# changhaonan/A3VLM

Hardware: AMD Instinct MI355X
Metric: image-text samples/sec (train) + articulation-decode tok/s (higher is better)
Workload: dtype bf16

## Files before the change

### a3vlm_amd/csrc/a3v_strip.hip

```cpp
#include "a3v_common.h"

namespace {
typedef __attribute__((ext_vector_type(4))) short s16x4;
constexpr int SBK = 64;
constexpr int SBN = 128;
constexpr int A_TILE = SBK * 128;
constexpr int W_TILE = SBK * 256;
constexpr int S_STAGE = A_TILE + W_TILE;

struct StripArgs {
  const bf16_t* T;
  const bf16_t* X;
  float* part;
  int64_t ldt, ldx;
  int R, N, Kt;
};

__device__ __forceinline__ int key_a(int k) { return (((k >> 3) & 1) << 1) | ((k >> 1) & 1); }
__device__ __forceinline__ int key_w(int k) { return (((k >> 3) & 1) << 2) | (k & 3); }

template <int NST>
__global__ __launch_bounds__(256) void gemm_tn_strip_kernel(StripArgs p) {
  __shared__ __attribute__((aligned(1024))) char lds[NST * S_STAGE];
  const int tid = threadIdx.x, lane = tid & 63;
  const int wave = __builtin_amdgcn_readfirstlane(tid >> 6);
  const int n0 = blockIdx.x * SBN;
  const int nk_all = (p.Kt + SBK - 1) / SBK;
  const int kt0 = (int)((int64_t)nk_all * blockIdx.y / gridDim.y), kt1 = (int)((int64_t)nk_all * (blockIdx.y + 1) / gridDim.y);
  const auto rsT = __builtin_amdgcn_make_buffer_rsrc((void*)p.T, 0, (int)(((int64_t)(p.Kt - 1) * p.ldt + 64) * 2), 0x00020000);
  const auto rsX = __builtin_amdgcn_make_buffer_rsrc((void*)p.X, 0, (int)(((int64_t)(p.Kt - 1) * p.ldx + p.N) * 2), 0x00020000);
  unsigned voT[2], voX[4];
#pragma unroll
  for (int c = 0; c < 2; ++c) {
    const int row = (wave * 2 + c) * 8 + (lane >> 3), pos = lane & 7;
    voT[c] = (unsigned)((row * p.ldt) * 2 + ((((pos >> 1) ^ key_a(row)) << 5) + (pos & 1) * 16));
  }
#pragma unroll
  for (int c = 0; c < 4; ++c) {
    const int row = (wave * 4 + c) * 4 + (lane >> 4), pos = lane & 15;
    voX[c] = (unsigned)((row * p.ldx) * 2 + ((((pos >> 1) ^ key_w(row)) << 5) + (pos & 1) * 16));
  }
  auto stage = [&](int t) {
    char* base = lds + ((t - kt0) % NST) * S_STAGE;
    const unsigned soT = (unsigned)(((int64_t)t * SBK * p.ldt) * 2);
    const unsigned soX = (unsigned)(((int64_t)t * SBK * p.ldx + n0) * 2);
#pragma unroll
    for (int c = 0; c < 2; ++c)
      __builtin_amdgcn_raw_ptr_buffer_load_lds(rsT, (__attribute__((address_space(3))) void*)(base + (wave * 2 + c) * 1024), 16, voT[c] + soT, 0, 0, 0);
#pragma unroll
    for (int c = 0; c < 4; ++c)
      __builtin_amdgcn_raw_ptr_buffer_load_lds(rsX, (__attribute__((address_space(3))) void*)(base + A_TILE + (wave * 4 + c) * 1024), 16, voX[c] + soX, 0, 0, 0);
  };
  const int fg = lane >> 4, il = lane & 15;
  int roA[2][2], kA[2][2], roW[2][2], kW[2][2];
#pragma unroll
  for (int ks = 0; ks < 2; ++ks)
#pragma unroll
    for (int jj = 0; jj < 2; ++jj) {
      const int k = ks * 32 + 8 * fg + 4 * jj + (il >> 2);
      roA[ks][jj] = k * 128 + (il & 3) * 8;
      kA[ks][jj] = key_a(k);
// ... 10 lines not shown
  };

  f32x4 acc[4][2];
#pragma unroll
  for (int i = 0; i < 4; ++i)
#pragma unroll
    for (int j = 0; j < 2; ++j) acc[i][j] = f32x4{0.f, 0.f, 0.f, 0.f};

  if (kt0 < kt1) stage(kt0);
  if (NST == 3 && kt0 + 1 < kt1) stage(kt0 + 1);
  for (int t = kt0; t < kt1; ++t) {
    if (NST == 3 && t + 1 < kt1) asm volatile("s_waitcnt vmcnt(6)" ::: "memory");
    else asm volatile("s_waitcnt vmcnt(0)" ::: "memory");
    __syncthreads();
    if (t + NST - 1 < kt1) stage(t + NST - 1);
    const char* At = lds + ((t - kt0) % NST) * S_STAGE;
    const char* Wt = At + A_TILE;
    bf16x8 af[2][4], wf[2][2];
#pragma unroll
    for (int ks = 0; ks < 2; ++ks) {
#pragma unroll
      for (int i = 0; i < 4; ++i) af[ks][i] = tr8(At, roA[ks][0], roA[ks][1], i ^ kA[ks][0], i ^ kA[ks][1]);
#pragma unroll
      for (int j = 0; j < 2; ++j) wf[ks][j] = tr8(Wt, roW[ks][0], roW[ks][1], (wave * 2 + j) ^ kW[ks][0], (wave * 2 + j) ^ kW[ks][1]);
    }
#pragma unroll
    for (int ks = 0; ks < 2; ++ks)
#pragma unroll
      for (int i = 0; i < 4; ++i)
#pragma unroll
        for (int j = 0; j < 2; ++j)
          acc[i][j] = __builtin_amdgcn_mfma_f32_16x16x32_bf16(wf[ks][j], af[ks][i], acc[i][j], 0, 0, 0);
  }
  float* plane = p.part + (int64_t)blockIdx.y * p.R * p.N;
#pragma unroll
  for (int i = 0; i < 4; ++i) {
    const int m = 16 * i + (lane & 15);
    if (m >= p.R) continue;
#pragma unroll
    for (int j = 0; j < 2; ++j) {
      const int n = n0 + 32 * wave + 16 * j + 4 * (lane >> 4);
      if (n + 4 <= p.N) *reinterpret_cast<f32x4*>(plane + (int64_t)m * p.N + n) = acc[i][j];
    }
  }
}
}

extern "C" int a3v_gemm_tn_strip(const void* T, int64_t ldt, const void* X, int64_t ldx, float* partial, int R, int N, int Kt, int S,
                                 void* stream) {
  if (!T || !X || !partial || R <= 0 || N <= 0 || Kt <= 0 || S < 1 || S > 64) return A3V_ERR_ARG;
  if (R > 64 || R % 4 || N % 4 || ldt % 8 || ldx % 8 || ldt < 64 || S > (Kt + SBK - 1) / SBK) return A3V_ERR_SHAPE;
  if (((int64_t)(Kt - 1) * ldt + 64) * 2 >= (1LL << 31) || ((int64_t)(Kt - 1) * ldx + N) * 2 >= (1LL << 31)) return A3V_ERR_SHAPE;
  if ((reinterpret_cast<uintptr_t>(T) | reinterpret_cast<uintptr_t>(X) | reinterpret_cast<uintptr_t>(partial)) & 15) return A3V_ERR_SHAPE;
  StripArgs p{(const bf16_t*)T, (const bf16_t*)X, partial, ldt, ldx, R, N, Kt};
  hipLaunchKernelGGL(gemm_tn_strip_kernel<2>, dim3((N + SBN - 1) / SBN, S), dim3(256), 0, (hipStream_t)stream, p);
  A3V_LAUNCH_CHECK();
  return A3V_OK;
}
```

### a3vlm_amd/lib.py

```python
from __future__ import annotations

import ctypes
import os
from ctypes import c_float, c_int, c_int64, c_void_p

_HERE = os.path.dirname(os.path.abspath(__file__))
LIB_PATH = os.environ.get("A3V_LIB_PATH") or os.path.join(_HERE, "liba3vlm_hip.so")

BF16, F32 = 0, 1
EPI_NONE, EPI_BIAS, EPI_GELU, EPI_QUICKGELU, EPI_RESIDUAL, EPI_SWIGLU, EPI_OUT_F32, EPI_RES_F32 = 0, 1, 2, 4, 8, 16, 32, 64
EPI_SWIGLU_BWD = 128

EPI_TILE_128, EPI_TILE_256, EPI_TILE_256PP = 1 << 16, 1 << 17, 1 << 18
EPI_TILE_192PP = 1 << 23

P, I, L, F = c_void_p, c_int, c_int64, c_float

SIGNATURES = {
    "a3v_version": (I, []),
    "a3v_reload_env": (I, []),
    "a3v_gemm_nt": (I, [P, L, P, L, P, L, I, I, I, P, P, L, I, I, P]),
    "a3v_gemm_qkv_rope": (I, [P, L, P, L, I, P, L, P, P, P, L, P, L, P, I, I, I, I, I, I, I, I, P]),
    "a3v_gemm_nt_fp8": (I, [P, L, P, P, L, P, P, L, I, I, I, P, P, L, I, P]),
    "a3v_gemm_qkv_rope_fp8": (I, [P, L, P, P, L, P, I, P, L, P, P, P, I, I, I, I, I, I, I, I, P]),
# ... 97 lines not shown
    "a3v_rope_kvcache_rows": (I, [P, L, P, L, P, P, P, P, I, I, I, I, I, I, P]),
    "a3v_attention_decode_rows": (I, [P, P, P, P, P, I, I, I, I, I, ctypes.POINTER(c_int64), P, P, I, P]),
    "a3v_attention_decode_rows_splits": (I, [I, I, I]),
    "a3v_attention_decode_rows_shared": (I, [P, P, P, P, P, P, P, I, I, I, I, I, ctypes.POINTER(c_int64), P, P, I, P]),
    "a3v_kv_copy_span": (I, [P, P, I, I, P, I, I, I, I, I, I, I, I, P]),
    "a3v_generate_step_rows": (I, [P, L, P, I, I, P, L, P, P, I, P, P, I, P, P, P, P, P, P]),
    "a3v_llama_decode_step_rows_form": (I, [I, I, I, I, I, I, I]),
    "a3v_rope_kvcache_spans": (I, [P, L, P, L, P, P, P, P, P, I, I, I, I, I, I, I, P]),
    "a3v_attention_verify_rows": (I, [P, P, P, P, P, P, I, I, I, I, I, I, ctypes.POINTER(c_int64), P, P, I, P]),
    "a3v_attention_verify_rows_splits": (I, [I, I, I]),
    "a3v_attention_verify_rows_scratch_floats": (L, [I, I, I, I, I]),
    "a3v_lookup_draft_rows": (I, [P, L, P, P, P, P, P, I, I, I, I, P, P, P]),
    "a3v_accept_rows": (I, [P, L, I, I, I, P, P, P, L, P, P, I, P, P, I, P, P, P, P, P, P]),
    "a3v_llama_decode_step_verify_form": (I, [I, I, I, I, I, I, I, I]),
    "a3v_seen_mark": (I, [P, L, P, P, L, I, I, P]),
    "a3v_seen_clear_rows": (I, [P, P, I, L, L, I, P]),
    "a3v_logits_prepare": (I, [P, L, P, L, F, P, L, P, I, I, P]),
    "a3v_generate_record": (I, [P, L, P, P, L, I, P, P, P, L, P, L, I, I, P, I, I, P]),
    "a3v_adam8_quantize": (I, [P, P, P, P, P, P, L, P]),
    "a3v_adam8_dequantize": (I, [P, P, P, P, P, P, L, P]),
    "a3v_adamw8_scaled": (I, [P, P, P, P, P, P, L, F, F, F, F, F, L, P, P, P]),
}

class LlamaLayer(ctypes.Structure):
    _fields_ = [(n, c_void_p) for n in ("attn_norm_w", "wqkv", "wo", "ffn_norm_w", "w13", "w2", "k_cache", "vt_cache",
                                        "wqkv_q", "wqkv_s", "wo_q", "wo_s", "w13_q", "w13_s", "w2_q", "w2_s",
                                        "wqkv_n4", "wqkv_n4s", "wo_n4", "wo_n4s", "w13_n4", "w13_n4s", "w2_n4", "w2_n4s")]


class Kv8Layer(ctypes.Structure):
    _fields_ = [(n, c_void_p) for n in ("k_q", "vt_q", "k_scale", "v_scale")]


class ImageDesc(ctypes.Structure):
    _fields_ = [("src", c_void_p), ("coeffs", c_void_p), ("bounds", c_void_p), ("H", c_int), ("W", c_int), ("side", c_int), ("pad_x", c_int),
                ("pad_y", c_int), ("ksize", c_int)]


SIGNATURES["a3v_llama_decode_step"] = (I, [ctypes.POINTER(LlamaLayer), I, P, P, P, P, P, P, P, P, I, I, I, I, I, I, I, I, F, P])
SIGNATURES["a3v_llama_decode_step_kv8"] = (I, [ctypes.POINTER(LlamaLayer), ctypes.POINTER(Kv8Layer), I, P, P, P, P, P, P, P, P, P, P,
                                               I, I, I, I, I, I, I, I, F, P])
SIGNATURES["a3v_llama_decode_step_form"] = (I, [I, I, I, I, I, I, I])
SIGNATURES["a3v_llama_decode_step_rows"] = (I, [ctypes.POINTER(LlamaLayer), I, P, P, P, P, P, P, P, P, P, I, I, I, I, I, I, I, I, F, P])
SIGNATURES["a3v_llama_decode_step_verify"] = (I, [ctypes.POINTER(LlamaLayer), I, P, P, P, P, P, P, P, P, P, P, I, I, I, I, I, I, I, I, I, F, P])
SIGNATURES["a3v_llama_decode_step_rows_shared"] = (I, [ctypes.POINTER(LlamaLayer), I, P, P, P, P, P, P, P, P, P, P, P, I, I, I, I, I, I, I, I,
                                                       F, P])

_lib = None


def load() -> ctypes.CDLL:
    global _lib
    if _lib is not None:
        return _lib
    if not os.path.isfile(LIB_PATH):
        raise RuntimeError(
            f"{LIB_PATH} not found: the HIP extension is not built. Run "
            "`python -c 'import __graft_entry__ as g; g.build()'` (or `make -C a3vlm_amd/csrc`). "
            "a3vlm_amd has no non-HIP fallback.")
    import torch
    lib = ctypes.CDLL(LIB_PATH)
    for name, (res, args) in SIGNATURES.items():
        fn = getattr(lib, name)
        fn.restype = res
        fn.argtypes = args
    _lib = lib
    return lib


class env:

    def __init__(self, **kw):
        self.kw = {k: str(v) for k, v in kw.items()}
        self.old = {}

    def __enter__(self):
        for k, v in self.kw.items():
            self.old[k] = os.environ.get(k)
            os.environ[k] = v
# ... 24 lines not shown
```

### a3vlm_amd/ops.py

```python
from __future__ import annotations

import ctypes
from typing import Optional

import torch

from . import lib as _l
from .lib import BF16, F32, EPI_BIAS, EPI_GELU, EPI_QUICKGELU, EPI_RESIDUAL, EPI_SWIGLU, EPI_OUT_F32, EPI_RES_F32, EPI_SWIGLU_BWD

_DT = {torch.bfloat16: BF16, torch.float32: F32}


def dt(t: torch.Tensor) -> int:
    try:
        return _DT[t.dtype]
    except KeyError:
        raise TypeError(f"a3vlm_amd supports bf16/fp32 tensors, got {t.dtype}")


def _p(t: Optional[torch.Tensor]):
    return None if t is None else t.data_ptr()


def _stream() -> int:
# ... 999 lines not shown


def grad_finish_multi(table, n_jobs: int, total_units: int, max_blocks: int = 0):
    _dev(table)
    assert table.dtype == torch.int64 and table.is_contiguous() and tuple(table.shape) == (n_jobs, 22)
    rc = _l.load().a3v_grad_finish_multi(_p(table), int(n_jobs), int(total_units), int(max_blocks), _stream())
    _l.check(rc, f"a3v_grad_finish_multi(jobs={n_jobs},units={total_units})")


def rmsnorm_bwd_parts(x, w, dy, dh, parts, eps, row_idx=None):
    _dev(x, w, dy, dh, parts, row_idx)
    assert w.dtype == torch.float32 and x.dtype == dh.dtype == dy.dtype == torch.bfloat16 and parts.dtype == torch.float32
    rows, dim = x.shape
    if row_idx is not None:
        assert row_idx.dtype == torch.int32 and row_idx.is_contiguous()
        rows = row_idx.numel()
        assert dy.shape[0] == rows
    assert parts.is_contiguous() and parts.numel() >= (rows + 7) // 8 * dim
    rc = _l.load().a3v_rmsnorm_bwd_parts_bf16(_p(x), x.stride(0), _p(row_idx), _p(w), _p(dy), dy.stride(0), _p(dh), dh.stride(0), _p(parts),
                                              rows, dim, eps, _stream())
    _l.check(rc, "a3v_rmsnorm_bwd_parts_bf16")


def gemm_tn_strip_planes(t, x, planes, S: int):
    _dev(t, x, planes)
    Kt, R = t.shape
    N = x.shape[1]
    assert x.shape[0] == Kt and t.stride(1) == 1 and x.stride(1) == 1 and t.stride(0) >= 64
    assert planes.dtype == torch.float32 and planes.is_contiguous() and planes.numel() >= S * R * N
    rc = _l.load().a3v_gemm_tn_strip(_p(t), t.stride(0), _p(x), x.stride(0), _p(planes), R, N, Kt, S, _stream())
    _l.check(rc, f"a3v_gemm_tn_strip(R={R},N={N},Kt={Kt},S={S})")


def lora_refresh(wa, wb, A, At, B, Bt, col0: int, row0: int):
    _dev(wa, wb, A, At, B, Bt)
    assert wa.dtype == torch.float32 and wb.dtype == torch.float32 and wa.is_contiguous() and wb.is_contiguous()
    assert all(t.dtype == torch.bfloat16 and t.stride(1) == 1 for t in (A, At, B, Bt))
    r, in_f = wa.shape
    nj = wb.shape[0]
    assert wb.shape[1] == r and col0 + r <= A.shape[0] and in_f <= A.shape[1] and row0 + nj <= B.shape[0]
    rc = _l.load().a3v_lora_refresh(_p(wa), _p(wb), r, in_f, nj, _p(A), A.stride(0), _p(At), At.stride(0), _p(B), B.stride(0), _p(Bt),
                                    Bt.stride(0), col0, row0, _stream())
    _l.check(rc, "a3v_lora_refresh")
```

### a3vlm_amd/train.py

```python
from __future__ import annotations

import os

from contextlib import contextmanager
from typing import Callable, Dict, List, Optional, Tuple

import torch

from . import grad_finish, ops
from .train_images import GROUPS, _AdapterImages, _Fp8Images, _Images, _Nf4Images, _pad64, group_modules
from .util import install_param_epoch_hook


def skinny_slices(M: int, N: int, K: int, cus: int) -> int:
    blocks = ((M + 127) // 128) * ((N + 127) // 128)
    nk = K // 64
    S = 1
    while blocks * S < 512 and S * 2 <= nk and S < 32:
        S *= 2
    if N <= 64 and M >= 2048 and cus > 0:
        S = max(1, min(cus // ((M + 255) // 256), nk // 2, 32))
    elif N <= 64 and M >= 512 and S > 4:
        S = 4
    return S


def label_rows_ref(labels: torch.Tensor, W: int, S: int):
    T = labels.shape[1]
    flat = labels.reshape(-1)
    pos = torch.nonzero(flat != 0).reshape(-1)
    b = torch.div(pos, T, rounding_mode="floor")
    return (b * S + W + (pos - b * T)).to(torch.int32), pos.to(torch.int32), flat[pos]


class TrainEngine:
    fuse_qkv_rope = os.environ.get("A3V_FUSE_QKV_ROPE", "1") != "0"
    tn_wgrad = os.environ.get("A3V_TN_WGRAD", "1") != "0"
    nn_dgrad = os.environ.get("A3V_NN_DGRAD", "1") != "0"
    packed_attn_bwd = os.environ.get("A3V_PACKED_ATTN_BWD", "1") != "0"
    lora_kext = os.environ.get("A3V_LORA_KEXT", "1") != "0"
    lora_nt_dgrad = os.environ.get("A3V_LORA_NT_DGRAD", "all")
    strip_wgrad = os.environ.get("A3V_STRIP_WGRAD", "1") != "0"
    fuse_swiglu_bwd = os.environ.get("A3V_FUSE_SWIGLU_BWD", "1") != "0"
    label_rows = os.environ.get("A3V_LABEL_ROWS", "1") != "0"
    finish_defer = os.environ.get("A3V_FINISH_DEFER", "1") != "0"
    finish_budget = int(float(os.environ.get("A3V_FINISH_BUDGET_MB", grad_finish.DEFAULT_BUDGET // 2 ** 20)) * 2 ** 20)

    def __init__(self, model, compute_dtype: torch.dtype = torch.bfloat16, recompute: Optional[bool] = None,
                 stream_dtype: Optional[torch.dtype] = None, zero1_world: int = 0):
        install_param_epoch_hook()
        self.m = model
        self.lora = int(getattr(model, "lora_rank", 0) or 0) > 0
        self.act = compute_dtype
        if stream_dtype is None:
            stream_dtype = torch.float32 if os.environ.get("A3V_STREAM_FP32", "0") == "1" else compute_dtype
        self.stream = stream_dtype
        self.recompute = recompute
        self._img = None
        self._ws: Dict[tuple, torch.Tensor] = {}
        self._flat: Optional[torch.Tensor] = None
        self._views: Dict[str, torch.Tensor] = {}
        self._ranges: List[Tuple[str, int, int]] = []
        self._fresh: set = set()
        self._gemm_written: set = set()
        self.on_layer_grads_ready: Optional[Callable[[str, int, int], None]] = None
        self.sumsq_sink = None
        self.static_grad_scale: Optional[float] = None
        self._saved = None
        self._weights_ready: Dict[str, torch.cuda.Event] = {}
        self.zero1_world = int(zero1_world or 0)
        if "A3V_NN_DGRAD" not in os.environ:
            self.nn_dgrad = bool(self.zero1_world)
        if self._q4base() and self.zero1_world:
            raise ValueError("ZeRO-1 shards compute-dtype base matrices; an NF4 base (quantize_base_weights) has none")
        if self._q8base():
            if self.zero1_world:
                raise ValueError("ZeRO-1 shards compute-dtype base matrices; an fp8 base (quantize_base_weights) has none")
            if compute_dtype != torch.bfloat16:
                raise ValueError(f"an fp8 base trains under the bf16 compute dtype (the products of its GEMMs are bf16); got {compute_dtype}")
        self._flat_params: Optional[torch.Tensor] = None
        self._z1: List[tuple] = []
        self._z1_fresh = True
        self._params: Dict[str, torch.nn.Parameter] = {}
        self._offs: Dict[str, Tuple[int, int]] = {}
        self._adapters = _AdapterImages(self)
        self._cu_count: Optional[int] = None
        self._nt_mem_checked = False
        self._opt_stepped = False
        self._dha_ready = False
        self._dh_full: Optional[torch.Tensor] = None
        self._sel_rows: Optional[Tuple[int, int]] = None
        self.bucket_overlap = False
        self._fin: Optional[grad_finish.GradFinisher] = None
        self._fin_mode: Optional[str] = None
        self._fin_hold: Optional[List[str]] = None

    def _buf(self, name, shape, dtype=None, zero=False):
        dtype = dtype or self.act
        if self._sel_rows is not None:
            return self._sel_buf(name, tuple(shape), dtype, zero)
        key = (name, tuple(shape), dtype)
        t = self._ws.get(key)
        if t is None:
            t = torch.empty(*shape, dtype=dtype, device=self.m._device)
            self._ws[key] = t
        if zero:
            t.zero_()
        return t

    def _sel_buf(self, name, shape, dtype, zero):
        n, cap = self._sel_rows
        name += ".sel"
        if shape[0] == n:
            key = (name, (cap,) + shape[1:], dtype)
            t = self._ws.get(key)
            if t is None:
                t = self._ws[key] = torch.empty(*key[1], dtype=dtype, device=self.m._device)
            t = t[:n]
        else:
            numel = 1
            for d in shape:
                numel *= d
            key = (name, "flat", dtype)
            t = self._ws.get(key)
            if t is None or t.numel() < numel:
                t = self._ws[key] = torch.empty(numel, dtype=dtype, device=self.m._device)
            t = t[:numel].view(shape)
        if zero:
# ... 260 lines not shown
        if tn_ok and self._strip_ok(dy, x):
            S = self._strip_slices(M, K)
            ops.gemm_tn_strip(dy, x, grad, self._buf("splitk", (S * N * K,), torch.float32), S, accumulate=not fresh)
            return
        if tn_ok and min(N, K) <= 64 and max(N, K) >= 256:
            blocks = ((N + 255) // 256) * ((K + 255) // 256)
            S = 1
            while blocks * S < 256 and S < 16 and 2 * S <= (M + 63) // 64:
                S *= 2
            ops.gemm_tn_splitk(dy, x, grad, self._buf("splitk", (S * N * K,), torch.float32), S, accumulate=not fresh)
            return
        Mp = _pad64(M)
        dyt = self._buf("wg_dyt" + tag, (N, Mp))
        xt = self._buf("wg_xt" + tag, (K, Mp))
        ops.transpose(dy, dyt, M, N, Mp)
        ops.transpose(x, xt, M, K, Mp)
        if min(N, K) <= 64:
            self._skinny(dyt, xt, grad, accumulate=not fresh)
        else:
            ops.gemm_nt(dyt, xt, grad, residual=None if fresh else grad,
                        epilogue=(ops.EPI_OUT_F32 if fresh else ops.EPI_RES_F32) if self.act == torch.bfloat16 else 0)

    def _strip_ok(self, dy: torch.Tensor, x: torch.Tensor) -> bool:
        N, K = dy.shape[1], x.shape[1]
        return bool(self.strip_wgrad and N <= 64 and N % 4 == 0 and K >= 256 and dy.stride(0) >= 64
                    and (dy.data_ptr() | x.data_ptr()) % 16 == 0)

    @staticmethod
    def _strip_slices(M: int, K: int) -> int:
        return max(1, min(64, (M + 63) // 64, -(-512 // ((K + 127) // 128))))

    def _fin_begin(self) -> None:
        self._fin_mode, self._fin_hold = None, None
        flat = self._flat
        if not (self.finish_defer and self.lora and not self.recompute and not self.zero1_world and not self.bucket_overlap
                and self.stream == torch.bfloat16 and self.act == torch.bfloat16 and flat is not None and flat.is_cuda):
            return
        if self._fin is None or self._fin.flat_ptr != flat.data_ptr() or self._fin.plan.budget_bytes != self.finish_budget:
            self._fin = grad_finish.GradFinisher(self.finish_budget, flat.data_ptr())
            self._fin_mode = "plan"
        elif self._fin.arena is not None:
            self._fin.pending = {}
            self._fin_mode, self._fin_hold = "defer", []

    def _fin_end(self) -> None:
        if self._fin_mode == "plan":
            self._fin.commit(self._flat.device)
        elif self._fin_mode == "defer":
            self._fin.launch()
        self._fin_mode = None
        held, self._fin_hold = self._fin_hold, None
        for bucket in held or ():
            self._notify(bucket)

    def _fin_slot(self, key, add, signature: tuple, count: int):
        if self._fin_mode == "plan":
            try:
                add(self._fin.plan)
            except ValueError:
                pass
            return None
        if self._fin_mode != "defer":
            return None
        slot = self._fin.plan.slots.get(key)
        if slot is None or slot.signature() != signature or count > slot.count_cap or key in self._fin.pending:
            return None
        return slot

    def _wgrad_deferred(self, key, dy: torch.Tensor, x: torch.Tensor, dst=None, scatter=None) -> bool:
        if self._fin_mode is None or self.act != torch.bfloat16 or not self.tn_wgrad or not self._strip_ok(dy, x):
            return False
        (M, N), K = dy.shape, x.shape[1]
        if dy.stride(0) % 8 or x.stride(0) % 8 or 2 * M * max(dy.stride(0), x.stride(0)) >= 2 ** 31:
            return False
        S, S_cap = self._strip_slices(M, K), self._strip_slices(1 << 30, K)
        if scatter is None:
            sig = (grad_finish.PLANES, N, K, (dst.data_ptr(),), dst.stride(0), True, 0, (), ())
            add = lambda plan: plan.add_planes(key, N, K, S_cap, dst.data_ptr(), dst.stride(0), True)
        else:
            r, views, row0s = scatter
            ptrs, njs = tuple(v.data_ptr() for v in views), tuple(int(v.shape[0]) for v in views)
            if not all(v.is_contiguous() and v.shape[1] == r for v in views):
                return False
            sig = (grad_finish.SCATTER, N, K, ptrs, 0, True, r, tuple(row0s), njs)
            add = lambda plan: plan.add_scatter(key, N, K, S_cap, r, ptrs, row0s, njs)
        slot = self._fin_slot(key, add, sig, S)
        if slot is None:
            return False
        ops.gemm_tn_strip_planes(dy, x, self._fin.slice_of(slot, S * N * K), S)
        self._fin.pending[key] = S
        return True

    def _norm_bwd(self, key, x: torch.Tensor, w: torch.Tensor, dy: torch.Tensor, dh: torch.Tensor, dw: Optional[torch.Tensor], eps: float,
                  dh_lowp: Optional[torch.Tensor] = None):
        rows, dim = x.shape
        if (self._fin_mode is not None and dw is not None and dh_lowp is None and x.dtype == torch.bfloat16 and dy.dtype == torch.bfloat16
                and dim % 4 == 0 and dim <= 8192 and x.stride(0) % 4 == 0 and dy.stride(0) % 4 == 0 and dh.stride(0) % 4 == 0
                and (x.data_ptr() | dh.data_ptr() | dy.data_ptr()) % 8 == 0 and w.data_ptr() % 16 == 0):
            nb = (rows + 7) // 8
            cap = max(nb, (self._sel_rows[1] + 7) // 8 if self._sel_rows is not None else 0)
            sig = (grad_finish.COLSUM, 0, dim, (dw.data_ptr(),), 0, True, 0, (), ())
            slot = self._fin_slot(key, lambda plan: plan.add_colsum(key, cap, dim, dw.data_ptr()), sig, nb)
            if slot is not None:
                ops.rmsnorm_bwd_parts(x, w, dy, dh, self._fin.slice_of(slot, nb * dim), eps)
                self._fin.pending[key] = nb
                return
        ops.rmsnorm_bwd(x, w, dy, dh, dw, eps, dh_lowp=dh_lowp)

    def _skinny(self, a: torch.Tensor, w: torch.Tensor, out: torch.Tensor, accumulate: bool = False):
        M, K = a.shape
        N = w.shape[0]
        S = skinny_slices(M, N, K, self._cus(a.device) if a.is_cuda else 0)
        if S == 1 or self.act != torch.bfloat16 or K % 64:
            ops.gemm_nt(a, w, out, residual=out if accumulate else None,
                        epilogue=(ops.EPI_RES_F32 if accumulate else ops.EPI_OUT_F32) if self._res_epi(out) else 0)
            return
        ops.gemm_nt_splitk(a, w, out, self._buf("splitk", (S * M * N,), torch.float32), S, accumulate)

    def _cus(self, dev) -> int:
        if self._cu_count is None:
            self._cu_count = int(torch.cuda.get_device_properties(dev).multi_processor_count)
        return self._cu_count

    def _dgrad_w(self, dy: torch.Tensor, key: str, out: torch.Tensor):
# ... 83 lines not shown

    def _group_bwd(self, i: int, kind: str, dy: torch.Tensor, dy_full: Optional[torch.Tensor], x: torch.Tensor, t: Optional[torch.Tensor],
                   dx: torch.Tensor, swiglu_gu: Optional[torch.Tensor] = None):
        key = f"{kind}.{i}"
        if dy_full is None:
            self._dgrad_w(dy, key, dx)
            if self.lora:
                self._lora_bwd(i, key, dy, x, t, dx)
            return
        dt = dy_full[:, dy.shape[1]:]
        self._dgrad(dy, self._lora_step_images()[key + ".Bt"], dt)
        im = self._images()
        if swiglu_gu is not None:
            ops.gemm_nt(dy_full, im[key + ".yT"], dx, residual=swiglu_gu, epilogue=ops.EPI_SWIGLU_BWD)
        elif self._nt_dgrad(key):
            ops.gemm_nt(dy_full, im[key + ".yT"], dx)
        else:
            ops.gemm_nn(dy_full, im[key + ".y"], dx)
        self._lora_bwd(i, key, dy, x, t, None, dt=dt)

    def _group_wgrad(self, i: int, kind: str, dy: torch.Tensor, x: torch.Tensor):
        names = tuple(f"layers.{i}.{sub}.weight" for sub in GROUPS[kind])
        if self._has(*names):
            self._wgrad(dy, x, self._gview(names[0], names[-1]), kind, names)

    def _lora_bwd(self, i: int, key: str, dy: torch.Tensor, x: torch.Tensor, t: torch.Tensor, dx: Optional[torch.Tensor], dt=None):
        m = self.m
        li = self._lora_step_images()
        r = m.lora_rank
        Bt, At = li[key + ".Bt"], li[key + ".At"]
        M, N = dy.shape
        Rp = t.shape[1]
        if dt is None:
            dt = self._buf("lora_dt", (M, Rp))
            self._dgrad(dy, Bt, dt)
        g = key.split(".")[0]
        names = GROUPS[g]
        vas = [self._views[f"layers.{i}.{nm}.lora_a.weight"] for nm in names]
        vbs = [self._views[f"layers.{i}.{nm}.lora_b.weight"] for nm in names]
        nr = len(names) * r
        row0s, row = [], 0
        for vb in vbs:
            row0s.append(row)
            row += vb.shape[0]
        gBt = None
        if not (t.is_cuda and nr % 4 == 0 and self._wgrad_deferred((i, g, "gB"), t[:, :nr], dy, scatter=(r, vbs, row0s))):
            gBt = self._buf("lora_gBt." + g, (Rp, N), torch.float32)
            self._wgrad(t, dy, gBt, "lb", store=True)
        adjacent = all(vas[j + 1].data_ptr() == vas[j].data_ptr() + 4 * vas[j].numel() for j in range(len(vas) - 1))
        if adjacent and dt.stride(0) % 8 == 0:
            off = (vas[0].data_ptr() - self._flat.data_ptr()) // 4
            gA = self._flat[off:off + nr * x.shape[1]].view(nr, x.shape[1])
            if not self._wgrad_deferred((i, g, "gA"), dt[:, :nr], x, dst=gA):
                self._wgrad(dt[:, :nr], x, gA, "la", store=False)
        else:
            gA = self._buf("lora_gA." + g, (Rp, x.shape[1]), torch.float32)
            self._wgrad(dt, x, gA, "la", store=True)
            for j, va in enumerate(vas):
                ops.add2d(va, gA[j * r:(j + 1) * r])
        if gBt is None:
            pass
        elif gBt.is_cuda:
            ops.lora_gb_scatter(gBt, r, vbs, row0s)
        else:
            for j, vb in enumerate(vbs):
                vb.add_(gBt[j * r:(j + 1) * r, row0s[j]:row0s[j] + vb.shape[0]].t())
# ... 67 lines not shown

    def _qkv_fwd(self, i: int, xn, xn_full, t, qkv, qrot, kc, vc, B: int, S: int, tag: str) -> Optional[torch.Tensor]:
        m, im, key = self.m, self._images(), f"qkv.{i}"
        H, Hkv, hd = m.n_heads, m.n_kv_heads, m.head_dim
        fused = self.act == torch.bfloat16 and hd in (64, 128) and xn.shape[0] > 16 and self.fuse_qkv_rope
        v_rows = qkv[:, (H + Hkv) * hd:]
        if fused and not self.lora:
            ops.gemm_qkv_rope(xn, im[key], qrot, kc, vc, m._cos_sin_dev(), B, S, H, Hkv, hd, 0, 0, v_rows=v_rows)
            return None
        if t is not None:
            self._lora_t(key, xn, tag, t)
            ops.gemm_qkv_rope(xn_full, im[key + ".x"], qrot, kc, vc, m._cos_sin_dev(), B, S, H, Hkv, hd, 0, 0, v_rows=v_rows)
            return t
        if fused and self._q8base():
            t = self._lora_t(key, xn, tag)
            ops.gemm_nt(t, self._lora_step_images()[key + ".B"], qkv)
            xq = self._buf("q8_x", tuple(xn.shape), torch.uint8)
            sx = self._buf("q8_sx", (xn.shape[0],), torch.float32)
            ops.quantize_rows_fp8(xn, xq, sx)
            ops.gemm_qkv_rope_fp8_train(xq, sx, im[key + ".q"], im[key + ".s"], qrot, kc, vc, m._cos_sin_dev(), B, S, H, Hkv, hd, 0, 0,
                                        v_rows=v_rows, delta=qkv)
            return t
        if fused:
            t = self._lora_t(key, xn, tag)
            ops.gemm_nt(t, self._lora_step_images()[key + ".B"], qkv)
            ops.gemm_qkv_rope(xn, im[key], qrot, kc, vc, m._cos_sin_dev(), B, S, H, Hkv, hd, 0, 0, v_rows=v_rows, delta=qkv)
            return t
        t = self._group_fwd(i, "qkv", xn, xn_full, None, qkv, tag=tag)
        ops.rope_kvcache(qkv, qrot, kc, vc, m._cos_sin_dev(), B, S, H, Hkv, hd, 0, 0)
        return t

    def _block_backward(self, i: int, h_in: torch.Tensor, dh: torch.Tensor, B: int, S: int):
        rows, dim = B * S, self.m.args.dim
        if not self._saved.get("kept"):
            self._images().recompute_backward(i)
        k = self._saved["kept"][i] if self._saved.get("kept") else self._block_forward(i, h_in, B, S, keep=True)
        kx = self._kx(rows)
        if self.stream == torch.bfloat16 and self.act == torch.bfloat16:
            dha, dha_full = dh, (self._dh_full if kx else None)
        else:
            dha, dha_full = self._dy_buf("dh_act", dim, f"w2.{i}", rows, kx)
        datt = self._tail_backward(i, k, dh, dha, dha_full)
        self._attn_backward(i, k, h_in, dh, dha, datt, B, S)

    def _last_block_backward_rows(self, i: int, h_in: torch.Tensor, dh: torch.Tensor, dh_sel: torch.Tensor, B: int, S: int, sel: dict):
        m, k = self.m, self._saved["kept"][i]
        rows, dim = B * S, m.args.dim
        kx = self._kx(rows)
        assert k["h_mid"].shape[0] == sel["n"]
        with self._sel_section(sel):
            datt_sel = self._tail_backward(i, k, dh_sel[:, :dim], dh_sel[:, :dim], dh_sel if kx else None)
        datt = ops.scatter_rows(datt_sel, sel["rows"], self._buf("datt", (rows, m.n_heads * m.head_dim)))
        ops.scatter_rows(dh_sel[:, :dim], sel["rows"], dh)
        self._attn_backward(i, k, h_in, dh, dh, datt, B, S)

    def _tail_backward(self, i: int, k: dict, dh: torch.Tensor, dha: torch.Tensor, dha_full: Optional[torch.Tensor]) -> torch.Tensor:
        m, a, im = self.m, self.m.args, self._images()
        H, hd, dim, F = m.n_heads, m.head_dim, a.dim, m.ffn
        rows = dha.shape[0]
        l = m.layers[i]
        lt = k["lt"]
        kx = dha_full is not None
        stream_lp = self.stream == torch.bfloat16 and self.act == torch.bfloat16
        fuse_cast = self.act == torch.bfloat16 and not stream_lp
        if not stream_lp and not (fuse_cast and self._dha_ready):
            ops.cast(dh, dha)
        self._dha_ready = False
        self._group_wgrad(i, "w2", dha, k["act"])
        dgu, dgu_full = self._dy_buf("dgu", 2 * F, f"w13.{i}", rows, kx)
        ft_epi = (not self.lora and self.fuse_swiglu_bwd and self.act == torch.bfloat16 and dim % 64 == 0 and F % 8 == 0
                  and dha.stride(0) % 8 == 0)
        if kx and self.fuse_swiglu_bwd and self._nt_dgrad(f"w2.{i}") and F % 8 == 0:
            self._group_bwd(i, "w2", dha, dha_full, k["act"], lt["w2"], dgu, swiglu_gu=k["gu"])
        elif (ft_epi and self.nn_dgrad and F >= 256 and 2 * rows * dha.stride(0) < 2 ** 31 and 2 * F * dim < 2 ** 31
              and tuple(im[f"w2.{i}"].shape) == (dim, F)):
            ops.gemm_nn(dha, im[f"w2.{i}"], dgu, residual=k["gu"], epilogue=ops.EPI_SWIGLU_BWD)
        elif ft_epi and not self.nn_dgrad and tuple(im[f"w2.{i}.t"].shape) == (F, dim):
            ops.gemm_nt(dha, im[f"w2.{i}.t"], dgu, residual=k["gu"], epilogue=ops.EPI_SWIGLU_BWD)
        else:
            dact = self._buf("dact", (rows, F))
            self._group_bwd(i, "w2", dha, dha_full, k["act"], lt["w2"], dact)
            ops.swiglu_bwd(k["gu"], dact, dgu, F, interleaved=False)
        self._group_wgrad(i, "w13", dgu, k["xn2"])
        dxn = self._buf("dxn", (rows, dim))
        self._group_bwd(i, "w13", dgu, dgu_full, k["xn2"], lt["w13"], dxn)
        self._norm_bwd((i, "ffn_norm"), k["h_mid"], l.ffn_norm.weight, dxn, dh, self._views.get(f"layers.{i}.ffn_norm.weight"), a.norm_eps,
                       dh_lowp=dha if fuse_cast else None)
        if not fuse_cast and not stream_lp:
            ops.cast(dh, dha)
        self._group_wgrad(i, "wo", dha, k["att_wo"])
        datt = self._buf("datt", (rows, H * hd))
        self._group_bwd(i, "wo", dha, dha_full, k["att_wo"], lt["wo"], datt)
        return datt

    def _attn_backward(self, i: int, k: dict, h_in: torch.Tensor, dh: torch.Tensor, dha: torch.Tensor, datt: torch.Tensor, B: int, S: int):
        m, a = self.m, self.m.args
        H, Hkv, hd, dim = m.n_heads, m.n_kv_heads, m.head_dim, a.dim
        rows = B * S
        kx = self._kx(rows)
        fuse_cast = self.act == torch.bfloat16 and self.stream != torch.bfloat16
        D = self._buf("attn_D", (B, S, H), torch.float32)
        qkv = k["qkv"]
        ld = qkv.stride(0)
        vrows = qkv[:, (H + Hkv) * hd:]
        spad = k["spad"]
        dqkv, dqkv_full = self._dy_buf("dqkv", (H + 2 * Hkv) * hd, f"qkv.{i}", rows, kx)
        if self.act == torch.bfloat16 and hd in (64, 128) and self.packed_attn_bwd:
            ops.attention_bwd_packed(k["qrot"], k["kc"], Hkv * spad * hd, spad * hd, vrows, S * ld, ld, hd, k["att"], datt, k["lse"], D,
                                     dqkv, m._cos_sin_dev(), B, S, H, Hkv, hd, True, 0)
        else:
            dq = self._buf("dq", (rows, H * hd))
            dk = self._buf("dk", (B, Hkv, S, hd))
            dv = self._buf("dv", (B, Hkv, S, hd))
            wsp = None
            if self.act == torch.bfloat16 and hd in (64, 128):
                wsp = self._buf("attn_bwd_ws", (ops.attention_bwd_workspace_bytes(B, S, H, Hkv, hd),), torch.uint8)
            att_c = k["att"] if k["att"].is_contiguous() else k["att"].contiguous()
            ops.attention_bwd(k["qrot"], k["kc"], Hkv * spad * hd, spad * hd, vrows, S * ld, ld, hd, att_c, datt, k["lse"], D,
                              dq, dk, dv, B, S, H, Hkv, hd, True, workspace=wsp)
            ops.rope_bwd_pack(dq, dk, dv, dqkv, m._cos_sin_dev(), B, S, H, Hkv, hd, 0)
        self._group_wgrad(i, "qkv", dqkv, k["xn"])
        dxn = self._buf("dxn", (rows, dim))
        self._group_bwd(i, "qkv", dqkv, dqkv_full, k["xn"], k["lt"]["qkv"], dxn)
        self._norm_bwd((i, "attention_norm"), h_in, m.layers[i].attention_norm.weight, dxn, dh,
                       self._views.get(f"layers.{i}.attention_norm.weight"), a.norm_eps, dh_lowp=dha if fuse_cast else None)
        self._dha_ready = fuse_cast

    def _label_rows_engine(self) -> bool:
        return bool(self.label_rows and not self.recompute and not self.zero1_world
                    and self.stream == torch.bfloat16 and self.act == torch.bfloat16)

    @staticmethod
    def _label_rows_take(n: int, rows: int) -> bool:
        return 0 < n < rows

    def _label_rows(self, lab: torch.Tensor, W: int, S: int) -> Optional[dict]:
        B, T = lab.shape
        srows = self._buf("sel_stream_rows", (B * T,), torch.int32)
        hrows = self._buf("sel_head_rows", (B * T,), torch.int32)
        labs = self._buf("sel_labels", (B * T,), torch.int64)
        n_valid = self._buf("n_valid", (1,), torch.int32)
        n = int(ops.label_rows(lab, W, S, srows, hrows, labs, n_valid))
        if not self._label_rows_take(n, B * S):
            return None
        return dict(n=n, cap=B * T, rows=srows[:n], head=hrows[:n], lab=labs[:n], n_valid=n_valid)

    @torch.no_grad()
    def forward_loss(self, examples: torch.Tensor, labels: torch.Tensor, image: Optional[torch.Tensor] = None,
                     qformer_feats=None, extra_feats=None) -> torch.Tensor:
        self._check_dtypes()
        self._adapters.checked = False
        self._sel_rows = None
        m, a = self.m, self.m.args
        B, T = examples.shape
        n_img = 0 if image is None else (len(image) if isinstance(image, (list, tuple)) else 1)
        W = m.words_per_image * n_img if n_img else 0
# ... 298 lines not shown
```

### include/a3vlm_hip.h

```cpp
#ifndef A3VLM_HIP_H
#define A3VLM_HIP_H

#include <stdint.h>

#ifdef __cplusplus
extern "C" {
#endif

enum { A3V_BF16 = 0, A3V_F32 = 1 };

enum {
  A3V_OK = 0,
  A3V_ERR_SHAPE = -1,
  A3V_ERR_DTYPE = -2,
  A3V_ERR_ARG = -3
};

enum {
  A3V_EPI_NONE = 0,
  A3V_EPI_BIAS = 1,
  A3V_EPI_GELU = 2,
  A3V_EPI_QUICKGELU = 4,
  A3V_EPI_RESIDUAL = 8,
  A3V_EPI_SWIGLU = 16,
// ... 336 lines not shown
                      int64_t v_sb, int64_t v_ss, int64_t v_sh, const void* out, const void* dout,
                      const float* lse, float* D, void* dq, void* dk, void* dv, void* workspace,
                      int B, int S, int H, int Hkv, int hd, int causal, int dtype, void* stream);
int a3v_attention_bwd_packed(const void* q, const void* k, int64_t k_sb, int64_t k_sh, const void* v, int64_t v_sb,
                             int64_t v_ss, int64_t v_sh, const void* out, int64_t ld_out, const void* dout, const float* lse, float* D,
                             void* dqkv, int64_t ld_qkv, const float* cos_sin, int rope_pos0, int B, int S, int H, int Hkv,
                             int hd, int causal, int dtype, void* stream);
int64_t a3v_attention_bwd_workspace_bytes(int B, int S, int H, int Hkv, int hd);
int a3v_attention_bwd_mfma(const void* q, const void* k, int64_t k_sb, int64_t k_sh, const void* v,
                           int64_t v_sb, int64_t v_ss, int64_t v_sh, const void* dout, const float* lse,
                           const float* D, void* dq, void* dk, void* dv, void* workspace, int B, int S,
                           int H, int Hkv, int hd, int causal, void* stream);

int a3v_add2d(void* dst, int64_t ld_dst, const void* src, int64_t ld_src, int rows, int cols, int dtype, void* stream);
int a3v_cast(const void* src, int64_t ld_src, int src_dtype, void* dst, int64_t ld_dst, int dst_dtype,
             int rows, int cols, void* stream);

int a3v_embed_bwd(const int64_t* tokens, int64_t ld_tok, const float* dh, float* dtable, int B, int T,
                  int W, int dim, int vocab, void* stream);

int a3v_rows_sum(const void* src, int64_t ld, const int32_t* row_idx, int n_rows, int dim, float* out,
                 int dtype, void* stream);

int a3v_adamw(float* param, const float* grad, float* exp_avg, float* exp_avg_sq, int64_t n, float lr, float beta1, float beta2,
              float eps, float weight_decay, int64_t step, void* bf16_image, void* stream);

int a3v_adamw_scaled(float* param, const float* grad, float* exp_avg, float* exp_avg_sq, int64_t n, float lr, float beta1, float beta2,
                     float eps, float weight_decay, int64_t step, void* bf16_image, const float* grad_scale, void* stream);

int a3v_lora_gb_scatter(const float* gbt, int64_t ld, int r, int n_mods, float* const* dst, const int* row0, const int* nj, void* stream);

int a3v_gemm_tn_strip(const void* T, int64_t ldt, const void* X, int64_t ldx, float* partial, int R, int N, int Kt, int S, void* stream);

int a3v_adamw_scaled_t(float* param, const float* grad, float* exp_avg, float* exp_avg_sq, int rows, int cols, float lr, float beta1,
                       float beta2, float eps, float weight_decay, int64_t step, void* bf16_image, void* bf16_image_t, int64_t ldt,
                       const float* grad_scale, void* stream);

typedef struct {
  float* p; const float* g; float* m; float* v;
  int64_t n, cols;
  void* d1; int64_t s1r, s1c;
  void* d2; int64_t s2r, s2c;
} a3v_adamw_tensor;
int a3v_adamw_multi(const a3v_adamw_tensor* table, int n_tensors, int64_t max_n, float lr, float beta1, float beta2, float eps,
                    float weight_decay, int64_t step, const float* grad_scale, void* stream);

int a3v_adam8_quantize(const float* m, const float* v, uint8_t* m_q, float* m_scale, uint8_t* r_q, float* r_scale, int64_t n,
                       void* stream);
int a3v_adam8_dequantize(const uint8_t* m_q, const float* m_scale, const uint8_t* r_q, const float* r_scale, float* m, float* v,
                         int64_t n, void* stream);
int a3v_adamw8_scaled(float* param, const float* grad, uint8_t* m_q, float* m_scale, uint8_t* r_q, float* r_scale, int64_t n, float lr,
                      float beta1, float beta2, float eps, float weight_decay, int64_t step, void* bf16_image, const float* grad_scale,
                      void* stream);

enum { A3V_FINISH_PLANES = 0, A3V_FINISH_SCATTER = 1, A3V_FINISH_COLSUM = 2 };
typedef struct {
  int64_t kind;
  const float* src;
  int64_t S, R, N;
  int64_t ldo, accumulate;
  int64_t r, n_mods;
  float* dst[4];
  int64_t row0[4], nj[4];
  int64_t unit0;
} a3v_finish_job;
int a3v_grad_finish_multi(const a3v_finish_job* table, int n_jobs, int64_t total_units, int max_blocks, void* stream);
// ... 22 lines not shown
```

Baseline: 36.56.

## Batch deferred LoRA strip weight-gradient GEMMs into one grouped launch

Refactors the strip GEMM kernel body into a device function and adds a grouped kernel that runs up to eight strip jobs in one launch. Jobs are ordered heaviest first and located by block offset. In deferred-finish mode, the trainer queues strip wgrad GEMMs and flushes them before dependent ops and at block boundaries. This cuts per-kernel launch overhead and lets small strip GEMMs fill the GPU together, at the cost of extra flush points and a block-lookup loop in every block.

After: 36.82 (median of 6 runs). About the same (+0.7%).

```diff
diff --git a/a3vlm_amd/csrc/a3v_strip.hip b/a3vlm_amd/csrc/a3v_strip.hip
--- a/a3vlm_amd/csrc/a3v_strip.hip
+++ b/a3vlm_amd/csrc/a3v_strip.hip
@@ -20,13 +20,12 @@
 __device__ __forceinline__ int key_w(int k) { return (((k >> 3) & 1) << 2) | (k & 3); }
 
 template <int NST>
-__global__ __launch_bounds__(256) void gemm_tn_strip_kernel(StripArgs p) {
-  __shared__ __attribute__((aligned(1024))) char lds[NST * S_STAGE];
+__device__ __forceinline__ void strip_tile(const StripArgs& p, const int bx, const int by, const int ny, char* lds) {
   const int tid = threadIdx.x, lane = tid & 63;
   const int wave = __builtin_amdgcn_readfirstlane(tid >> 6);
-  const int n0 = blockIdx.x * SBN;
+  const int n0 = bx * SBN;
   const int nk_all = (p.Kt + SBK - 1) / SBK;
-  const int kt0 = (int)((int64_t)nk_all * blockIdx.y / gridDim.y), kt1 = (int)((int64_t)nk_all * (blockIdx.y + 1) / gridDim.y);
+  const int kt0 = (int)((int64_t)nk_all * by / ny), kt1 = (int)((int64_t)nk_all * (by + 1) / ny);
   const auto rsT = __builtin_amdgcn_make_buffer_rsrc((void*)p.T, 0, (int)(((int64_t)(p.Kt - 1) * p.ldt + 64) * 2), 0x00020000);
   const auto rsX = __builtin_amdgcn_make_buffer_rsrc((void*)p.X, 0, (int)(((int64_t)(p.Kt - 1) * p.ldx + p.N) * 2), 0x00020000);
   unsigned voT[2], voX[4];
@@ -103,7 +102,7 @@
         for (int j = 0; j < 2; ++j)
           acc[i][j] = __builtin_amdgcn_mfma_f32_16x16x32_bf16(wf[ks][j], af[ks][i], acc[i][j], 0, 0, 0);
   }
-  float* plane = p.part + (int64_t)blockIdx.y * p.R * p.N;
+  float* plane = p.part + (int64_t)by * p.R * p.N;
 #pragma unroll
   for (int i = 0; i < 4; ++i) {
     const int m = 16 * i + (lane & 15);
@@ -115,16 +114,123 @@
     }
   }
 }
-}
-
-extern "C" int a3v_gemm_tn_strip(const void* T, int64_t ldt, const void* X, int64_t ldx, float* partial, int R, int N, int Kt, int S,
-                                 void* stream) {
+
+template <int NST>
+__global__ __launch_bounds__(256) void gemm_tn_strip_kernel(StripArgs p) {
+  __shared__ __attribute__((aligned(1024))) char lds[NST * S_STAGE];
+  strip_tile<NST>(p, blockIdx.x, blockIdx.y, gridDim.y, lds);
+}
+
+struct StripGroupArgs {
+  StripArgs job[A3V_STRIP_MAX_JOBS];
+  int block0[A3V_STRIP_MAX_JOBS + 1];
+  int slices[A3V_STRIP_MAX_JOBS];
+  int n;
+};
+
+__host__ __device__ inline int strip_col_tiles(int N) { return (N + SBN - 1) / SBN; }
+
+__host__ __device__ inline void strip_group_locate(const int* block0, const int* ntiles, int n, int b, int* i, int* bx, int* by) {
+  int k = 0;
+  for (int q = 1; q < n; ++q)
+    if (b >= block0[q]) k = q;
+  const int lb = b - block0[k];
+  *i = k;
+  *bx = lb % ntiles[k];
+  *by = lb / ntiles[k];
+}
+
+template <int NST>
+__global__ __launch_bounds__(256) void gemm_tn_strip_group_kernel(StripGroupArgs g) {
+  __shared__ __attribute__((aligned(1024))) char lds[NST * S_STAGE];
+  int ntiles[A3V_STRIP_MAX_JOBS];
+#pragma unroll
+  for (int q = 0; q < A3V_STRIP_MAX_JOBS; ++q) ntiles[q] = q < g.n ? strip_col_tiles(g.job[q].N) : 1;
+  int i, bx, by;
+  strip_group_locate(g.block0, ntiles, g.n, (int)blockIdx.x, &i, &bx, &by);
+  const StripArgs p = g.job[i];
+  strip_tile<NST>(p, bx, by, g.slices[i], lds);
+}
+
+int strip_job_check(const void* T, int64_t ldt, const void* X, int64_t ldx, const float* partial, int R, int N, int Kt, int S) {
   if (!T || !X || !partial || R <= 0 || N <= 0 || Kt <= 0 || S < 1 || S > 64) return A3V_ERR_ARG;
   if (R > 64 || R % 4 || N % 4 || ldt % 8 || ldx % 8 || ldt < 64 || S > (Kt + SBK - 1) / SBK) return A3V_ERR_SHAPE;
   if (((int64_t)(Kt - 1) * ldt + 64) * 2 >= (1LL << 31) || ((int64_t)(Kt - 1) * ldx + N) * 2 >= (1LL << 31)) return A3V_ERR_SHAPE;
   if ((reinterpret_cast<uintptr_t>(T) | reinterpret_cast<uintptr_t>(X) | reinterpret_cast<uintptr_t>(partial)) & 15) return A3V_ERR_SHAPE;
+  return A3V_OK;
+}
+
+int strip_group_plan(const a3v_strip_job* jobs, int n_jobs, int* order, int* block0) {
+  if (!jobs || n_jobs < 1 || n_jobs > A3V_STRIP_MAX_JOBS) return A3V_ERR_ARG;
+  int64_t weight[A3V_STRIP_MAX_JOBS];
+  for (int j = 0; j < n_jobs; ++j) {
+    const a3v_strip_job& b = jobs[j];
+    if (b.N <= 0 || b.Kt <= 0 || b.S < 1 || b.S > 64) return A3V_ERR_ARG;
+    if (b.S > (b.Kt + SBK - 1) / SBK) return A3V_ERR_SHAPE;
+    weight[j] = (int64_t)((b.Kt + SBK - 1) / SBK) * strip_col_tiles(b.N);
+    order[j] = j;
+  }
+  for (int a = 1; a < n_jobs; ++a)
+    for (int q = a; q > 0 && weight[order[q]] > weight[order[q - 1]]; --q) { const int t = order[q]; order[q] = order[q - 1]; order[q - 1] = t; }
+  int64_t blocks = 0;
+  for (int i = 0; i < n_jobs; ++i) {
+    block0[i] = (int)blocks;
+    blocks += (int64_t)strip_col_tiles(jobs[order[i]].N) * jobs[order[i]].S;
+    if (blocks >= (1LL << 31)) return A3V_ERR_SHAPE;
+  }
+  block0[n_jobs] = (int)blocks;
+  return (int)blocks;
+}
+}
+
+extern "C" int a3v_gemm_tn_strip(const void* T, int64_t ldt, const void* X, int64_t ldx, float* partial, int R, int N, int Kt, int S,
+                                 void* stream) {
+  const int rc = strip_job_check(T, ldt, X, ldx, partial, R, N, Kt, S);
+  if (rc != A3V_OK) return rc;
   StripArgs p{(const bf16_t*)T, (const bf16_t*)X, partial, ldt, ldx, R, N, Kt};
   hipLaunchKernelGGL(gemm_tn_strip_kernel<2>, dim3((N + SBN - 1) / SBN, S), dim3(256), 0, (hipStream_t)stream, p);
   A3V_LAUNCH_CHECK();
   return A3V_OK;
 }
+
+extern "C" int a3v_gemm_tn_strip_multi(const a3v_strip_job* jobs, int n_jobs, void* stream) {
+  if (!jobs || n_jobs < 1 || n_jobs > A3V_STRIP_MAX_JOBS) return A3V_ERR_ARG;
+  for (int j = 0; j < n_jobs; ++j) {
+    const a3v_strip_job& b = jobs[j];
+    const int rc = strip_job_check(b.T, b.ldt, b.X, b.ldx, b.planes, b.R, b.N, b.Kt, b.S);
+    if (rc != A3V_OK) return rc;
+  }
+  StripGroupArgs g{};
+  int order[A3V_STRIP_MAX_JOBS];
+  const int blocks = strip_group_plan(jobs, n_jobs, order, g.block0);
+  if (blocks < 0) return blocks;
+  for (int i = 0; i < n_jobs; ++i) {
+    const a3v_strip_job& b = jobs[order[i]];
+    g.job[i] = StripArgs{(const bf16_t*)b.T, (const bf16_t*)b.X, b.planes, b.ldt, b.ldx, b.R, b.N, b.Kt};
+    g.slices[i] = b.S;
+  }
+  g.n = n_jobs;
+  hipLaunchKernelGGL(gemm_tn_strip_group_kernel<2>, dim3((unsigned)blocks), dim3(256), 0, (hipStream_t)stream, g);
+  A3V_LAUNCH_CHECK();
+  return A3V_OK;
+}
+
+extern "C" int a3v_strip_group_plan(const a3v_strip_job* jobs, int n_jobs, int32_t* order, int32_t* block0) {
+  if (!order || !block0) return A3V_ERR_ARG;
+  return strip_group_plan(jobs, n_jobs, order, block0);
+}
+
+extern "C" int a3v_strip_group_locate(const a3v_strip_job* jobs, int n_jobs, int block, int32_t* where) {
+  int order[A3V_STRIP_MAX_JOBS], block0[A3V_STRIP_MAX_JOBS + 1], ntiles[A3V_STRIP_MAX_JOBS];
+  if (!where) return A3V_ERR_ARG;
+  const int blocks = strip_group_plan(jobs, n_jobs, order, block0);
+  if (blocks < 0) return blocks;
+  if (block < 0 || block >= blocks) return A3V_ERR_ARG;
+  for (int i = 0; i < n_jobs; ++i) ntiles[i] = strip_col_tiles(jobs[order[i]].N);
+  int i, bx, by;
+  strip_group_locate(block0, ntiles, n_jobs, block, &i, &bx, &by);
+  where[0] = order[i];
+  where[1] = bx;
+  where[2] = by;
+  return A3V_OK;
+}
diff --git a/a3vlm_amd/lib.py b/a3vlm_amd/lib.py
--- a/a3vlm_amd/lib.py
+++ b/a3vlm_amd/lib.py
@@ -153,6 +153,14 @@
     _fields_ = [(n, c_void_p) for n in ("k_q", "vt_q", "k_scale", "v_scale")]
 
 
+class StripJob(ctypes.Structure):
+    _fields_ = [("T", c_void_p), ("ldt", c_int64), ("X", c_void_p), ("ldx", c_int64), ("planes", c_void_p),
+                ("R", ctypes.c_int32), ("N", ctypes.c_int32), ("Kt", ctypes.c_int32), ("S", ctypes.c_int32)]
+
+
+STRIP_MAX_JOBS = 8
+
+
 class ImageDesc(ctypes.Structure):
     _fields_ = [("src", c_void_p), ("coeffs", c_void_p), ("bounds", c_void_p), ("H", c_int), ("W", c_int), ("side", c_int), ("pad_x", c_int),
                 ("pad_y", c_int), ("ksize", c_int)]
@@ -166,6 +174,10 @@
 SIGNATURES["a3v_llama_decode_step_verify"] = (I, [ctypes.POINTER(LlamaLayer), I, P, P, P, P, P, P, P, P, P, P, I, I, I, I, I, I, I, I, I, F, P])
 SIGNATURES["a3v_llama_decode_step_rows_shared"] = (I, [ctypes.POINTER(LlamaLayer), I, P, P, P, P, P, P, P, P, P, P, P, I, I, I, I, I, I, I, I,
                                                        F, P])
+
+SIGNATURES["a3v_gemm_tn_strip_multi"] = (I, [ctypes.POINTER(StripJob), I, P])
+SIGNATURES["a3v_strip_group_plan"] = (I, [ctypes.POINTER(StripJob), I, ctypes.POINTER(ctypes.c_int32), ctypes.POINTER(ctypes.c_int32)])
+SIGNATURES["a3v_strip_group_locate"] = (I, [ctypes.POINTER(StripJob), I, I, ctypes.POINTER(ctypes.c_int32)])
 
 _lib = None
 
diff --git a/a3vlm_amd/ops.py b/a3vlm_amd/ops.py
--- a/a3vlm_amd/ops.py
+++ b/a3vlm_amd/ops.py
@@ -1055,6 +1055,37 @@
     _l.check(rc, f"a3v_gemm_tn_strip(R={R},N={N},Kt={Kt},S={S})")
 
 
+def strip_job(t, x, planes, S: int) -> tuple:
+    _dev(t, x, planes)
+    Kt, R = t.shape
+    N = x.shape[1]
+    assert t.dtype == x.dtype == torch.bfloat16
+    assert x.shape[0] == Kt and t.stride(1) == 1 and x.stride(1) == 1 and t.stride(0) >= 64
+    assert planes.dtype == torch.float32 and planes.is_contiguous() and planes.numel() >= S * R * N
+    return (_p(t), t.stride(0), _p(x), x.stride(0), _p(planes), R, N, Kt, int(S))
+
+
+def gemm_tn_strip_multi(jobs):
+    n = len(jobs)
+    assert 1 <= n <= _l.STRIP_MAX_JOBS
+    tab = (_l.StripJob * n)(*jobs)
+    _l.check(_l.load().a3v_gemm_tn_strip_multi(tab, n, _stream()), f"a3v_gemm_tn_strip_multi(jobs={n})")
+
+
+def strip_group_map(shapes):
+    n = len(shapes)
+    tab = (_l.StripJob * n)(*[(None, 0, None, 0, None, 0, int(N), int(Kt), int(S)) for N, Kt, S in shapes])
+    order, block0, where = (ctypes.c_int32 * n)(), (ctypes.c_int32 * (n + 1))(), (ctypes.c_int32 * 3)()
+    blocks = _l.load().a3v_strip_group_plan(tab, n, order, block0)
+    if blocks < 0:
+        _l.check(blocks, "a3v_strip_group_plan")
+    out = []
+    for b in range(blocks):
+        _l.check(_l.load().a3v_strip_group_locate(tab, n, b, where), "a3v_strip_group_locate")
+        out.append(tuple(where))
+    return list(order), list(block0), out
+
+
 def lora_refresh(wa, wb, A, At, B, Bt, col0: int, row0: int):
     _dev(wa, wb, A, At, B, Bt)
     assert wa.dtype == torch.float32 and wb.dtype == torch.float32 and wa.is_contiguous() and wb.is_contiguous()
diff --git a/a3vlm_amd/train.py b/a3vlm_amd/train.py
--- a/a3vlm_amd/train.py
+++ b/a3vlm_amd/train.py
@@ -7,7 +7,7 @@
 
 import torch
 
-from . import grad_finish, ops
+from . import grad_finish, lib, ops
 from .train_images import GROUPS, _AdapterImages, _Fp8Images, _Images, _Nf4Images, _pad64, group_modules
 from .util import install_param_epoch_hook
 
@@ -44,6 +44,7 @@
     fuse_swiglu_bwd = os.environ.get("A3V_FUSE_SWIGLU_BWD", "1") != "0"
     label_rows = os.environ.get("A3V_LABEL_ROWS", "1") != "0"
     finish_defer = os.environ.get("A3V_FINISH_DEFER", "1") != "0"
+    strip_group = os.environ.get("A3V_STRIP_GROUP", "1") != "0"
     finish_budget = int(float(os.environ.get("A3V_FINISH_BUDGET_MB", grad_finish.DEFAULT_BUDGET // 2 ** 20)) * 2 ** 20)
 
     def __init__(self, model, compute_dtype: torch.dtype = torch.bfloat16, recompute: Optional[bool] = None,
@@ -94,6 +95,7 @@
         self._fin: Optional[grad_finish.GradFinisher] = None
         self._fin_mode: Optional[str] = None
         self._fin_hold: Optional[List[str]] = None
+        self._strip_queue: List[tuple] = []
 
     def _buf(self, name, shape, dtype=None, zero=False):
         dtype = dtype or self.act
@@ -420,6 +422,7 @@
 
     def _fin_begin(self) -> None:
         self._fin_mode, self._fin_hold = None, None
+        self._strip_queue = []
         flat = self._flat
         if not (self.finish_defer and self.lora and not self.recompute and not self.zero1_world and not self.bucket_overlap
                 and self.stream == torch.bfloat16 and self.act == torch.bfloat16 and flat is not None and flat.is_cuda):
@@ -435,6 +438,7 @@
         if self._fin_mode == "plan":
             self._fin.commit(self._flat.device)
         elif self._fin_mode == "defer":
+            self._strip_flush()
             self._fin.launch()
         self._fin_mode = None
         held, self._fin_hold = self._fin_hold, None
@@ -475,9 +479,22 @@
         slot = self._fin_slot(key, add, sig, S)
         if slot is None:
             return False
-        ops.gemm_tn_strip_planes(dy, x, self._fin.slice_of(slot, S * N * K), S)
+        planes = self._fin.slice_of(slot, S * N * K)
+        if self._fin_mode == "defer" and self.strip_group:
+            if len(self._strip_queue) == lib.STRIP_MAX_JOBS:
+                self._strip_flush()
+            self._strip_queue.append((dy, x, planes, S))
+        else:
+            ops.gemm_tn_strip_planes(dy, x, planes, S)
         self._fin.pending[key] = S
         return True
+
+    def _strip_flush(self) -> None:
+        q, self._strip_queue = self._strip_queue, []
+        if len(q) == 1:
+            ops.gemm_tn_strip_planes(*q[0])
+        elif q:
+            ops.gemm_tn_strip_multi([ops.strip_job(*j) for j in q])
 
     def _norm_bwd(self, key, x: torch.Tensor, w: torch.Tensor, dy: torch.Tensor, dh: torch.Tensor, dw: Optional[torch.Tensor], eps: float,
                   dh_lowp: Optional[torch.Tensor] = None):
@@ -627,6 +644,7 @@
         M, N = dy.shape
         Rp = t.shape[1]
         if dt is None:
+            self._strip_flush()
             dt = self._buf("lora_dt", (M, Rp))
             self._dgrad(dy, Bt, dt)
         g = key.split(".")[0]
@@ -760,6 +778,7 @@
 
     def _block_backward(self, i: int, h_in: torch.Tensor, dh: torch.Tensor, B: int, S: int):
         rows, dim = B * S, self.m.args.dim
+        self._strip_flush()
         if not self._saved.get("kept"):
             self._images().recompute_backward(i)
         k = self._saved["kept"][i] if self._saved.get("kept") else self._block_forward(i, h_in, B, S, keep=True)
@@ -774,6 +793,7 @@
     def _last_block_backward_rows(self, i: int, h_in: torch.Tensor, dh: torch.Tensor, dh_sel: torch.Tensor, B: int, S: int, sel: dict):
         m, k = self.m, self._saved["kept"][i]
         rows, dim = B * S, m.args.dim
+        self._strip_flush()
         kx = self._kx(rows)
         assert k["h_mid"].shape[0] == sel["n"]
         with self._sel_section(sel):
@@ -812,6 +832,7 @@
         self._group_wgrad(i, "w13", dgu, k["xn2"])
         dxn = self._buf("dxn", (rows, dim))
         self._group_bwd(i, "w13", dgu, dgu_full, k["xn2"], lt["w13"], dxn)
+        self._strip_flush()
         self._norm_bwd((i, "ffn_norm"), k["h_mid"], l.ffn_norm.weight, dxn, dh, self._views.get(f"layers.{i}.ffn_norm.weight"), a.norm_eps,
                        dh_lowp=dha if fuse_cast else None)
         if not fuse_cast and not stream_lp:
@@ -850,6 +871,7 @@
         self._group_wgrad(i, "qkv", dqkv, k["xn"])
         dxn = self._buf("dxn", (rows, dim))
         self._group_bwd(i, "qkv", dqkv, dqkv_full, k["xn"], k["lt"]["qkv"], dxn)
+        self._strip_flush()
         self._norm_bwd((i, "attention_norm"), h_in, m.layers[i].attention_norm.weight, dxn, dh,
                        self._views.get(f"layers.{i}.attention_norm.weight"), a.norm_eps, dh_lowp=dha if fuse_cast else None)
         self._dha_ready = fuse_cast
diff --git a/include/a3vlm_hip.h b/include/a3vlm_hip.h
--- a/include/a3vlm_hip.h
+++ b/include/a3vlm_hip.h
@@ -392,6 +392,19 @@
 
 int a3v_gemm_tn_strip(const void* T, int64_t ldt, const void* X, int64_t ldx, float* partial, int R, int N, int Kt, int S, void* stream);
 
+#define A3V_STRIP_MAX_JOBS 8
+typedef struct {
+  const void* T;
+  int64_t ldt;
+  const void* X;
+  int64_t ldx;
+  float* planes;
+  int32_t R, N, Kt, S;
+} a3v_strip_job;
+int a3v_gemm_tn_strip_multi(const a3v_strip_job* jobs, int n_jobs, void* stream);
+int a3v_strip_group_plan(const a3v_strip_job* jobs, int n_jobs, int32_t* order, int32_t* block0);
+int a3v_strip_group_locate(const a3v_strip_job* jobs, int n_jobs, int block, int32_t* where);
+
 int a3v_adamw_scaled_t(float* param, const float* grad, float* exp_avg, float* exp_avg_sq, int rows, int cols, float lr, float beta1,
                        float beta2, float eps, float weight_decay, int64_t step, void* bf16_image, void* bf16_image_t, int64_t ldt,
                        const float* grad_scale, void* stream);
```
